# theouterlimitz/Audio-Mastering-Engine

Measured on AMD Instinct MI355X. Metric: mastered Msamples/sec (48 kHz stereo f32) at 1/2/4/8 GPUs; % HBM roofline, higher is better.
Workload: dtype f64

## Files before the change

audio-mastering-engine_amd/csrc/amx_scan.hip:

```cpp
#include "amx_dev.hpp"

namespace amx {

typedef double d2s __attribute__((ext_vector_type(2)));

template <int D, int GP, bool DOWN>
__global__ void __launch_bounds__(AMX_BLOCK) k_scan_blk(const ScanBlk *__restrict__ blks,
                                                        int n_blk, const double *__restrict__ e,
                                                        double *__restrict__ s,
                                                        const double *__restrict__ M,
                                                        const double *__restrict__ Mbk, int K,
                                                        const double *__restrict__ carry,
                                                        double *__restrict__ eb,
                                                        const double *__restrict__ tailP,
                                                        double *__restrict__ tail) {
    static_assert(GP >= D && GP <= 64, "group fits a wave");
    constexpr int GW = 64 / GP;
    constexpr int GPB = GW * (AMX_BLOCK / 64);
    __shared__ __attribute__((aligned(16))) double lds[AMX_BLOCK];
    __shared__ __attribute__((aligned(16))) double s_pow[DOWN ? AMX_SCAN_PW * D * D : 1];
    const int t = threadIdx.x, w = t >> 6, l = t & 63;
    if constexpr (DOWN) {
        const int np = (K - 1 < AMX_SCAN_PW ? K - 1 : AMX_SCAN_PW) * D * D;
        for (int k = t; k < np; k += AMX_BLOCK) s_pow[k] = Mbk[k];
        __syncthreads();
    }
    const int gl = l / GP, i = l % GP;
    const bool lane_ok = gl < GW;
    const int64_t g = (int64_t)blockIdx.x * GPB + w * GW + (lane_ok ? gl : 0);
    const bool gvalid = lane_ok && g < 2LL * n_blk;
    const int b = gvalid ? (int)(g >> 1) : 0;
    const int ch = (int)(g & 1);
    const ScanBlk bk = blks[b];
    const bool row = lane_ok && i < D;
    const int ri = row ? i : 0;
    double mrow[D];
#pragma unroll
    for (int k = 0; k < D; k++) mrow[k] = row ? M[i * D + k] : 0.0;
    const int n = gvalid && (DOWN || !bk.last) ? bk.nseg : 0;
    double ev[AMX_SCAN_S];
#pragma unroll
    for (int q = 0; q < AMX_SCAN_S; q++) {
        const int qq = q < n ? q : 0;
        const int64_t jj = (int64_t)bk.seg0 + qq;
        ev[q] = e[(jj * 2 + ch) * D + ri];
    }
    double *my = lds + w * 64 + (lane_ok ? gl * GP : 0);
    double v = 0.0;
    if constexpr (DOWN) {
        auto xin = [&](int bb) -> double {
            if (bb == bk.first)
                return carry ? carry[((int64_t)bk.stream * 2 + ch) * D + ri] : 0.0;
            return eb[((int64_t)(bb - 1) * 2 + ch) * D + ri];
        };
        v = (gvalid && row) ? xin(b) : 0.0;
        double xs[AMX_SCAN_PW + 1];
#pragma unroll
        for (int k = 1; k <= AMX_SCAN_PW; k++) {
            const int bb = b - k;
            xs[k] = (k < K && gvalid && bb >= bk.first && row) ? xin(bb) : 0.0;
        }
        for (int k = 1; k < K; k++) {
            const int bb = b - k;
            const bool ok = gvalid && bb >= bk.first;
            double xk = 0.0;
#pragma unroll
            for (int q = 1; q <= AMX_SCAN_PW; q++) xk = q == k ? xs[q] : xk;
            if (lane_ok) my[i] = k <= AMX_SCAN_PW ? xk : ((ok && row) ? xin(bb) : 0.0);
            __builtin_amdgcn_wave_barrier();
            const double *P = (k <= AMX_SCAN_PW ? s_pow : Mbk) + ((int64_t)(k - 1) * D + ri) * D;
            double a0 = 0.0, a1 = 0.0;
#pragma unroll
            for (int m = 0; m < D; m += 2) {
                a0 = fma(P[m], my[m], a0);
                if (m + 1 < D) a1 = fma(P[m + 1], my[m + 1], a1);
            }
            __builtin_amdgcn_wave_barrier();
            if (ok && row) v += a0 + a1;
        }
    }
#pragma unroll
    for (int q = 0; q < AMX_SCAN_S; q++) {
        if (q >= n) break;
        if (DOWN) {
            const int64_t jj = (int64_t)bk.seg0 + q;
            if (row) s[(jj * 2 + ch) * D + i] = v;
            if (q == n - 1) {
                if constexpr (D == AMX_KW_DIM) {
                    if (tail && bk.last) {
                        if (lane_ok) my[i] = v;
                        __builtin_amdgcn_wave_barrier();
                        double acc = 0.0;
#pragma unroll
                        for (int qq = 0; qq < AMX_SCAN_S; qq++) acc = qq == q ? ev[qq] : acc;
                        const double *Pt = tailP + (int64_t)bk.stream * 16;
#pragma unroll
                        for (int k = 0; k < D; k++) acc = fma(Pt[ri * 4 + k], my[k], acc);
                        if (row) tail[((int64_t)bk.stream * 2 + ch) * D + i] = acc;
                        __builtin_amdgcn_wave_barrier();
                    }
                }
                break;
            }
        }
        if (lane_ok) my[i] = v;
        __builtin_amdgcn_wave_barrier();
        double a0 = row ? ev[q] : 0.0, a1 = 0.0, a2 = 0.0, a3 = 0.0;
        double mv[D];
#pragma unroll
        for (int k = 0; k < D; k += 2) {
            if (k + 1 < D) {
                const d2s pr = *reinterpret_cast<const d2s *>(my + k);
                mv[k] = pr.x;
                mv[k + 1] = pr.y;
            } else {
                mv[k] = my[k];
            }
        }
#pragma unroll
        for (int k = 0; k < D; k += 4) {
            a0 = fma(mrow[k], mv[k], a0);
            if (k + 1 < D) a1 = fma(mrow[k + 1], mv[k + 1], a1);
            if (k + 2 < D) a2 = fma(mrow[k + 2], mv[k + 2], a2);
            if (k + 3 < D) a3 = fma(mrow[k + 3], mv[k + 3], a3);
        }
        __builtin_amdgcn_wave_barrier();
        v = (a0 + a1) + (a2 + a3);
    }
    if (!DOWN && n > 0 && row) eb[((int64_t)b * 2 + ch) * D + i] = v;
}

template <int D, int GP>
static hipError_t scan_t(const ScanPlan &p, const double *e, double *s, const double *carry,
                         double *eb, bool up, const double *tailP, double *tail, hipStream_t st) {
    constexpr int GPB = (64 / GP) * (AMX_BLOCK / 64);
    const dim3 gb((unsigned)((2 * (int64_t)p.n_blk + GPB - 1) / GPB));
    if (up)
        hipLaunchKernelGGL((k_scan_blk<D, GP, false>), gb, dim3(AMX_BLOCK), 0, st, p.blks, p.n_blk, e,
                           s, p.M, p.Mbk, p.K, carry, eb, nullptr, nullptr);
    hipLaunchKernelGGL((k_scan_blk<D, GP, true>), gb, dim3(AMX_BLOCK), 0, st, p.blks, p.n_blk, e,
                       s, p.M, p.Mbk, p.K, carry, eb, tailP, tail);
    return hipGetLastError();
}

hipError_t launch_scan(const ScanPlan &p, const double *e, double *s, const double *carry,
                       double *eb, hipStream_t st, bool up, const double *tailP, double *tail) {
    if (p.n_blk <= 0 || p.D <= 0) return hipSuccess;
    if (tail && p.D != AMX_KW_DIM) return hipErrorInvalidValue;
    switch (p.D) {
    case 2: return scan_t<2, 2>(p, e, s, carry, eb, up, tailP, tail, st);
    case 4: return scan_t<4, 4>(p, e, s, carry, eb, up, tailP, tail, st);
    case 8: return scan_t<8, 8>(p, e, s, carry, eb, up, tailP, tail, st);
    case 10: return scan_t<10, 10>(p, e, s, carry, eb, up, tailP, tail, st);
    case 12: return scan_t<12, 12>(p, e, s, carry, eb, up, tailP, tail, st);
    case 16: return scan_t<16, 16>(p, e, s, carry, eb, up, tailP, tail, st);
    case 18: return scan_t<18, 18>(p, e, s, carry, eb, up, tailP, tail, st);
    case 20: return scan_t<20, 20>(p, e, s, carry, eb, up, tailP, tail, st);
    }
    return hipErrorInvalidValue;
}

}
```

Baseline: 31290.

## Fuse up-sweep and down-sweep scan into one kernel with recomputed halo blocks

Replaces the two-kernel block scan (up-sweep writing block carries to global, then down-sweep reading them) with a single fused kernel. Each workgroup takes a run of R blocks plus a K-block halo, recomputes the halo block end-states into shared memory, and then does the K-term carry combination and down-sweep from LDS. This removes one kernel launch and the global round trip for block carries, at the cost of redundant halo computation and extra LDS use. The non-up path keeps a separate down-only kernel.

After: 31580 (median of 5 runs). Within noise of the previous version (+0.9%).

```diff
diff --git a/audio-mastering-engine_amd/csrc/amx_scan.hip b/audio-mastering-engine_amd/csrc/amx_scan.hip
--- a/audio-mastering-engine_amd/csrc/amx_scan.hip
+++ b/audio-mastering-engine_amd/csrc/amx_scan.hip
@@ -4,23 +4,104 @@
 
 typedef double d2s __attribute__((ext_vector_type(2)));
 
-template <int D, int GP, bool DOWN>
-__global__ void __launch_bounds__(AMX_BLOCK) k_scan_blk(const ScanBlk *__restrict__ blks,
-                                                        int n_blk, const double *__restrict__ e,
-                                                        double *__restrict__ s,
-                                                        const double *__restrict__ M,
-                                                        const double *__restrict__ Mbk, int K,
-                                                        const double *__restrict__ carry,
-                                                        double *__restrict__ eb,
-                                                        const double *__restrict__ tailP,
-                                                        double *__restrict__ tail) {
+
+template <int D>
+__device__ __forceinline__ double scan_step(const double (&mrow)[D], double *my, int i, bool lane_ok,
+                                            bool row, double v, double eq) {
+    if (lane_ok) my[i] = v;
+    __builtin_amdgcn_wave_barrier();
+    double a0 = row ? eq : 0.0, a1 = 0.0, a2 = 0.0, a3 = 0.0;
+    double mv[D];
+#pragma unroll
+    for (int k = 0; k < D; k += 2) {
+        if (k + 1 < D) {
+            const d2s pr = *reinterpret_cast<const d2s *>(my + k);
+            mv[k] = pr.x;
+            mv[k + 1] = pr.y;
+        } else {
+            mv[k] = my[k];
+        }
+    }
+#pragma unroll
+    for (int k = 0; k < D; k += 4) {
+        a0 = fma(mrow[k], mv[k], a0);
+        if (k + 1 < D) a1 = fma(mrow[k + 1], mv[k + 1], a1);
+        if (k + 2 < D) a2 = fma(mrow[k + 2], mv[k + 2], a2);
+        if (k + 3 < D) a3 = fma(mrow[k + 3], mv[k + 3], a3);
+    }
+    __builtin_amdgcn_wave_barrier();
+    return (a0 + a1) + (a2 + a3);
+}
+
+template <int D>
+__device__ __forceinline__ double scan_wterm(const double *P, double *my, int i, bool lane_ok, double xk) {
+    if (lane_ok) my[i] = xk;
+    __builtin_amdgcn_wave_barrier();
+    double a0 = 0.0, a1 = 0.0;
+#pragma unroll
+    for (int m = 0; m < D; m += 2) {
+        a0 = fma(P[m], my[m], a0);
+        if (m + 1 < D) a1 = fma(P[m + 1], my[m + 1], a1);
+    }
+    __builtin_amdgcn_wave_barrier();
+    return a0 + a1;
+}
+
+template <int D>
+__device__ __forceinline__ void scan_tail(const double *Pt, double *my, int i, int ri, bool lane_ok,
+                                          bool row, double v, double e_last, double *out) {
+    if (lane_ok) my[i] = v;
+    __builtin_amdgcn_wave_barrier();
+    double acc = e_last;
+#pragma unroll
+    for (int k = 0; k < D; k++) acc = fma(Pt[ri * 4 + k], my[k], acc);
+    if (row) out[i] = acc;
+    __builtin_amdgcn_wave_barrier();
+}
+
+template <int D>
+__device__ __forceinline__ void scan_down(const double (&mrow)[D], const double (&ev)[AMX_SCAN_S],
+                                          double *my, int i, int ri, bool lane_ok, bool row, double v,
+                                          int n, const ScanBlk &bk, int ch, double *__restrict__ s,
+                                          const double *__restrict__ tailP, double *__restrict__ tail) {
+#pragma unroll
+    for (int q = 0; q < AMX_SCAN_S; q++) {
+        if (q >= n) break;
+        const int64_t jj = (int64_t)bk.seg0 + q;
+        if (row) s[(jj * 2 + ch) * D + i] = v;
+        if (q == n - 1) {
+            if constexpr (D == AMX_KW_DIM) {
+                if (tail && bk.last) {
+                    double el = 0.0;
+#pragma unroll
+                    for (int qq = 0; qq < AMX_SCAN_S; qq++) el = qq == q ? ev[qq] : el;
+                    scan_tail<D>(tailP + (int64_t)bk.stream * 16, my, i, ri, lane_ok, row, v, el,
+                                 tail + ((int64_t)bk.stream * 2 + ch) * D);
+                }
+            }
+            break;
+        }
+        v = scan_step<D>(mrow, my, i, lane_ok, row, v, ev[q]);
+    }
+}
+
+template <int D, int GP>
+__global__ void __launch_bounds__(AMX_BLOCK) k_scan_down(const ScanBlk *__restrict__ blks,
+                                                         int n_blk, const double *__restrict__ e,
+                                                         double *__restrict__ s,
+                                                         const double *__restrict__ M,
+                                                         const double *__restrict__ Mbk, int K,
+                                                         const double *__restrict__ carry,
+                                                         const double *__restrict__ eb,
+                                                         const double *__restrict__ tailP,
+                                                         double *__restrict__ tail) {
     static_assert(GP >= D && GP <= 64, "group fits a wave");
     constexpr int GW = 64 / GP;
     constexpr int GPB = GW * (AMX_BLOCK / 64);
     __shared__ __attribute__((aligned(16))) double lds[AMX_BLOCK];
-    __shared__ __attribute__((aligned(16))) double s_pow[DOWN ? AMX_SCAN_PW * D * D : 1];
+    __shared__ __attribute__((aligned(16))) double s_pow[AMX_SCAN_PW * D * D];
     const int t = threadIdx.x, w = t >> 6, l = t & 63;
-    if constexpr (DOWN) {
+    {
         const int np = (K - 1 < AMX_SCAN_PW ? K - 1 : AMX_SCAN_PW) * D * D;
         for (int k = t; k < np; k += AMX_BLOCK) s_pow[k] = Mbk[k];
         __syncthreads();
@@ -37,7 +118,7 @@
     double mrow[D];
 #pragma unroll
     for (int k = 0; k < D; k++) mrow[k] = row ? M[i * D + k] : 0.0;
-    const int n = gvalid && (DOWN || !bk.last) ? bk.nseg : 0;
+    const int n = gvalid ? bk.nseg : 0;
     double ev[AMX_SCAN_S];
 #pragma unroll
     for (int q = 0; q < AMX_SCAN_S; q++) {
@@ -46,100 +127,131 @@
         ev[q] = e[(jj * 2 + ch) * D + ri];
     }
     double *my = lds + w * 64 + (lane_ok ? gl * GP : 0);
-    double v = 0.0;
-    if constexpr (DOWN) {
+    auto xin = [&](int bb) -> double {
+        if (bb == bk.first)
+            return carry ? carry[((int64_t)bk.stream * 2 + ch) * D + ri] : 0.0;
+        return eb[((int64_t)(bb - 1) * 2 + ch) * D + ri];
+    };
+    double v = (gvalid && row) ? xin(b) : 0.0;
+    double xs[AMX_SCAN_PW + 1];
+#pragma unroll
+    for (int k = 1; k <= AMX_SCAN_PW; k++) {
+        const int bb = b - k;
+        xs[k] = (k < K && gvalid && bb >= bk.first && row) ? xin(bb) : 0.0;
+    }
+    for (int k = 1; k < K; k++) {
+        const int bb = b - k;
+        const bool ok = gvalid && bb >= bk.first;
+        double xk = 0.0;
+#pragma unroll
+        for (int q = 1; q <= AMX_SCAN_PW; q++) xk = q == k ? xs[q] : xk;
+        if (k > AMX_SCAN_PW) xk = (ok && row) ? xin(bb) : 0.0;
+        const double *P = (k <= AMX_SCAN_PW ? s_pow : Mbk) + ((int64_t)(k - 1) * D + ri) * D;
+        const double a = scan_wterm<D>(P, my, i, lane_ok, xk);
+        if (ok && row) v += a;
+    }
+    scan_down<D>(mrow, ev, my, i, ri, lane_ok, row, v, n, bk, ch, s, tailP, tail);
+}
+
+template <int D, int GP>
+__global__ void __launch_bounds__(AMX_BLOCK) k_scan_fused(const ScanBlk *__restrict__ blks,
+                                                          int n_blk, const double *__restrict__ e,
+                                                          double *__restrict__ s,
+                                                          const double *__restrict__ M,
+                                                          const double *__restrict__ Mbk, int K,
+                                                          const double *__restrict__ carry,
+                                                          double *__restrict__ eb,
+                                                          const double *__restrict__ tailP,
+                                                          double *__restrict__ tail, int R) {
+    static_assert(GP >= D && GP <= 64, "group fits a wave");
+    constexpr int GW = 64 / GP;
+    constexpr int GPB = GW * (AMX_BLOCK / 64);
+    constexpr int RB = GPB / 2;
+    static_assert(GPB % 2 == 0, "a block's two channels share a pass");
+    __shared__ __attribute__((aligned(16))) double lds[AMX_BLOCK];
+    __shared__ __attribute__((aligned(16))) double s_pow[AMX_SCAN_PW * D * D];
+    extern __shared__ __attribute__((aligned(16))) double s_E[];
+    const int t = threadIdx.x, w = t >> 6, l = t & 63;
+    {
+        const int np = (K - 1 < AMX_SCAN_PW ? K - 1 : AMX_SCAN_PW) * D * D;
+        for (int k = t; k < np; k += AMX_BLOCK) s_pow[k] = Mbk[k];
+    }
+    const int b0 = (int)blockIdx.x * R;
+    const int b1 = b0 + R < n_blk ? b0 + R : n_blk;
+    const int base = b0 - K;
+    const int first0 = blks[b0].first;
+    const int lo = first0 > base ? first0 : base;
+    const int gl = l / GP, i = l % GP;
+    const bool lane_ok = gl < GW;
+    const int slot = w * GW + (lane_ok ? gl : 0);
+    const int ch = slot & 1;
+    const bool row = lane_ok && i < D;
+    const int ri = row ? i : 0;
+    double mrow[D];
+#pragma unroll
+    for (int k = 0; k < D; k++) mrow[k] = row ? M[i * D + k] : 0.0;
+    double *my = lds + w * 64 + (lane_ok ? gl * GP : 0);
+    for (int p = base; p < b1; p += RB) {
+        const int bs = p + (slot >> 1);
+        const bool gvalid = lane_ok && bs >= lo && bs < b1;
+        const bool own = gvalid && bs >= b0;
+        const int b = gvalid ? bs : b0;
+        const ScanBlk bk = blks[b];
+        const int n = gvalid ? bk.nseg : 0;
+        double ev[AMX_SCAN_S];
+#pragma unroll
+        for (int q = 0; q < AMX_SCAN_S; q++) {
+            const int qq = q < n ? q : 0;
+            const int64_t jj = (int64_t)bk.seg0 + qq;
+            ev[q] = e[(jj * 2 + ch) * D + ri];
+        }
+        const int nu = bk.last ? 0 : n;
+        double v = 0.0;
+#pragma unroll
+        for (int q = 0; q < AMX_SCAN_S; q++) {
+            if (q >= nu) break;
+            v = scan_step<D>(mrow, my, i, lane_ok, row, v, ev[q]);
+        }
+        if (nu > 0 && row) {
+            s_E[((b - base) * 2 + ch) * D + i] = v;
+            if (own) eb[((int64_t)b * 2 + ch) * D + i] = v;
+        }
+        __syncthreads();
         auto xin = [&](int bb) -> double {
             if (bb == bk.first)
                 return carry ? carry[((int64_t)bk.stream * 2 + ch) * D + ri] : 0.0;
-            return eb[((int64_t)(bb - 1) * 2 + ch) * D + ri];
+            return s_E[((bb - 1 - base) * 2 + ch) * D + ri];
         };
-        v = (gvalid && row) ? xin(b) : 0.0;
-        double xs[AMX_SCAN_PW + 1];
-#pragma unroll
-        for (int k = 1; k <= AMX_SCAN_PW; k++) {
-            const int bb = b - k;
-            xs[k] = (k < K && gvalid && bb >= bk.first && row) ? xin(bb) : 0.0;
-        }
+        v = (own && row) ? xin(b) : 0.0;
         for (int k = 1; k < K; k++) {
             const int bb = b - k;
-            const bool ok = gvalid && bb >= bk.first;
-            double xk = 0.0;
-#pragma unroll
-            for (int q = 1; q <= AMX_SCAN_PW; q++) xk = q == k ? xs[q] : xk;
-            if (lane_ok) my[i] = k <= AMX_SCAN_PW ? xk : ((ok && row) ? xin(bb) : 0.0);
-            __builtin_amdgcn_wave_barrier();
+            const bool ok = own && bb >= bk.first;
+            const double xk = (ok && row) ? xin(bb) : 0.0;
             const double *P = (k <= AMX_SCAN_PW ? s_pow : Mbk) + ((int64_t)(k - 1) * D + ri) * D;
-            double a0 = 0.0, a1 = 0.0;
-#pragma unroll
-            for (int m = 0; m < D; m += 2) {
-                a0 = fma(P[m], my[m], a0);
-                if (m + 1 < D) a1 = fma(P[m + 1], my[m + 1], a1);
-            }
-            __builtin_amdgcn_wave_barrier();
-            if (ok && row) v += a0 + a1;
-        }
-    }
-#pragma unroll
-    for (int q = 0; q < AMX_SCAN_S; q++) {
-        if (q >= n) break;
-        if (DOWN) {
-            const int64_t jj = (int64_t)bk.seg0 + q;
-            if (row) s[(jj * 2 + ch) * D + i] = v;
-            if (q == n - 1) {
-                if constexpr (D == AMX_KW_DIM) {
-                    if (tail && bk.last) {
-                        if (lane_ok) my[i] = v;
-                        __builtin_amdgcn_wave_barrier();
-                        double acc = 0.0;
-#pragma unroll
-                        for (int qq = 0; qq < AMX_SCAN_S; qq++) acc = qq == q ? ev[qq] : acc;
-                        const double *Pt = tailP + (int64_t)bk.stream * 16;
-#pragma unroll
-                        for (int k = 0; k < D; k++) acc = fma(Pt[ri * 4 + k], my[k], acc);
-                        if (row) tail[((int64_t)bk.stream * 2 + ch) * D + i] = acc;
-                        __builtin_amdgcn_wave_barrier();
-                    }
-                }
-                break;
-            }
-        }
-        if (lane_ok) my[i] = v;
-        __builtin_amdgcn_wave_barrier();
-        double a0 = row ? ev[q] : 0.0, a1 = 0.0, a2 = 0.0, a3 = 0.0;
-        double mv[D];
-#pragma unroll
-        for (int k = 0; k < D; k += 2) {
-            if (k + 1 < D) {
-                const d2s pr = *reinterpret_cast<const d2s *>(my + k);
-                mv[k] = pr.x;
-                mv[k + 1] = pr.y;
-            } else {
-                mv[k] = my[k];
-            }
-        }
-#pragma unroll
-        for (int k = 0; k < D; k += 4) {
-            a0 = fma(mrow[k], mv[k], a0);
-            if (k + 1 < D) a1 = fma(mrow[k + 1], mv[k + 1], a1);
-            if (k + 2 < D) a2 = fma(mrow[k + 2], mv[k + 2], a2);
-            if (k + 3 < D) a3 = fma(mrow[k + 3], mv[k + 3], a3);
-        }
-        __builtin_amdgcn_wave_barrier();
-        v = (a0 + a1) + (a2 + a3);
-    }
-    if (!DOWN && n > 0 && row) eb[((int64_t)b * 2 + ch) * D + i] = v;
+            const double a = scan_wterm<D>(P, my, i, lane_ok, xk);
+            if (ok && row) v += a;
+        }
+        scan_down<D>(mrow, ev, my, i, ri, lane_ok, row, v, own ? n : 0, bk, ch, s, tailP, tail);
+    }
 }
 
 template <int D, int GP>
 static hipError_t scan_t(const ScanPlan &p, const double *e, double *s, const double *carry,
                          double *eb, bool up, const double *tailP, double *tail, hipStream_t st) {
     constexpr int GPB = (64 / GP) * (AMX_BLOCK / 64);
-    const dim3 gb((unsigned)((2 * (int64_t)p.n_blk + GPB - 1) / GPB));
-    if (up)
-        hipLaunchKernelGGL((k_scan_blk<D, GP, false>), gb, dim3(AMX_BLOCK), 0, st, p.blks, p.n_blk, e,
-                           s, p.M, p.Mbk, p.K, carry, eb, nullptr, nullptr);
-    hipLaunchKernelGGL((k_scan_blk<D, GP, true>), gb, dim3(AMX_BLOCK), 0, st, p.blks, p.n_blk, e,
-                       s, p.M, p.Mbk, p.K, carry, eb, tailP, tail);
+    if (up) {
+        constexpr int RB = GPB / 2;
+        const int K = p.K > 1 ? p.K : 1;
+        const int NB = ((13 * K + 2) / 3 + RB - 1) / RB * RB;
+        const int R = NB - K;
+        const dim3 gf((unsigned)((p.n_blk + R - 1) / R));
+        hipLaunchKernelGGL((k_scan_fused<D, GP>), gf, dim3(AMX_BLOCK), sizeof(double) * 2 * D * NB, st,
+                           p.blks, p.n_blk, e, s, p.M, p.Mbk, K, carry, eb, tailP, tail, R);
+    } else {
+        const dim3 gb((unsigned)((2 * (int64_t)p.n_blk + GPB - 1) / GPB));
+        hipLaunchKernelGGL((k_scan_down<D, GP>), gb, dim3(AMX_BLOCK), 0, st, p.blks, p.n_blk, e, s,
+                           p.M, p.Mbk, p.K, carry, eb, tailP, tail);
+    }
     return hipGetLastError();
 }
 
```
